# nadimkanazi/cacto

Measured on AMD Instinct MI355X. Metric: env-steps/sec + critic-updates/sec per node, double_integrator & manipulator, higher is better.
Workload: dtype f32 (MLP, MFMA) / f64 (dynamics)

## Files before the change

### cacto_amd/csrc/rollout_kernels.hip

```cpp
#include <cstdlib>
#include <utility>

#include "net_common.h"

#ifdef CACTO_STAMPS
__device__ unsigned long long g_rstamps[20];
__device__ unsigned long long g_ttacc[1024 * 2 * 2 * 10];
__device__ unsigned long long g_wsacc[1024 * 8 * 7];
#define RSTAMP(k)                                                                     \
  do {                                                                                \
    if (blockIdx.x == 0 && threadIdx.x == 0 && it == 20) g_rstamps[k] = __builtin_amdgcn_s_memtime(); \
  } while (0)
#else
#define RSTAMP(k) \
  do {            \
  } while (0)
#endif

namespace cacto {

template <typename F, int... I>
__device__ __forceinline__ void static_for_impl(F&& f, std::integer_sequence<int, I...>) {
  (f(std::integral_constant<int, I>{}), ...);
}
// ... 884 lines not shown
        const double* s = sr.s;
#pragma unroll
        for (int i = 0; i < na; ++i) {
          a[i] = use_actor ? Sh.W.a[c * na + i] : 0.f;
          ad[i] = (double)a[i];
        }
        if constexpr (NJ > 0) {
          if (split_dyn) {
            double M[NJ * NJ], h[NJ];
#pragma unroll
            for (int k = 0; k < NJ * NJ; ++k) M[k] = Sh.MS[k * SL + c];
#pragma unroll
            for (int i = 0; i < NJ; ++i) h[i] = Sh.hS[i * SL + c];
            chain_step<NJ>(sd, s, ad, M, h, sn);
          } else if (NJ == 3 && planar) {
            planar3_step(Planar3(sd.pl), ks.dt, s, ad, sn);
          } else {
            ro_simulate<NJ>(ks, sr.cd, s, ad, sn);
          }
        } else {
          ro_simulate<NJ>(ks, sr.cd, s, ad, sn);
        }
        RSTAMP(6);
#pragma unroll
        for (int i = 0; i < ns; ++i) {
          Sh.sS[c * ns + i] = sn[i];
          sr.s[i] = sn[i];
        }
      }
      constexpr bool EARLY = NJ >= 3;
      if constexpr (EARLY) {
        __builtin_amdgcn_fence(__ATOMIC_ACQ_REL, "wavefront");
        x0l.write(Sh, nrm, L.lane);
      }
      RSTAMP(16);
      if (active) {
        fin = ro_advance<NJ, NG>(c, sr.b, sr.t, sr.s, a, sd, T, Straj, Atraj, status, nrm, sr.n);
        sr.t += 1;
        RSTAMP(7);
      }
      ro_refill<NJ, NG>(fin, c, head, Sh, sd, S0, nsteps, order, T, B, G, Straj, status, nrm, L, (int)blockIdx.x);
      if (fin) sr.load(Sh, c, cdyn);
      if constexpr (!EARLY) {
        __builtin_amdgcn_fence(__ATOMIC_ACQ_REL, "wavefront");
        x0l.write(Sh, nrm, L.lane);
      }
      const uint64_t m = __ballot(L.lane < SL && Sh.sact[c]);
      if (L.lane == 0) Sh.anyact = m != 0;
      RSTAMP(8);
    }
    __syncthreads();
    RSTAMP(3);
  }
}

struct RoSplitTT {
  static constexpr int REGK = 128, LDSK = 128;
};

template <int NA>
struct RoTeamActorLds {
  static constexpr int SL = 4;
  float h1[4 * RoCfg<1>::H1B];
  float h2[SL * RoCfg<1>::H2S];
  float x0[64];
  float a[SL * NA];
};

template <int NJ>
struct RoTeamShared {
  static constexpr int ns = Dims<NJ>::NS, na = Dims<NJ>::NA, SL = 4;
  RoTeamActorLds<na> W;
  double sS[SL * ns];
  double MS[NJ > 0 ? SL * NJ * NJ : 1], hS[NJ > 0 ? SL * NJ : 1];
  int sb[SL], sn[SL], st[SL], sact[SL];
  int anyact;
  int bar;
};

template <int NJ>
struct RoTTShared {
  static constexpr int na = Dims<NJ>::NA;
  float4 w2[RoSplitTT::LDSK / 4 * 4 * 64];
  float w3[na * 256];
  float b3[8];
  RoTeamShared<NJ> team[2];
};

template <int NA>
struct RoTeamView {
  const float4* w2;
  const float* w3;
  const float* b3;
  float* h1;
  float* h2;
  float* x0;
  float* a;
};

#ifndef RO_TBAR_SLEEP
#define RO_TBAR_SLEEP 1
#endif
struct RoTeamBar {
  int* ctr;
  int target;
  int lane;
  __device__ __forceinline__ void operator()() {
    target += 4;
    if (lane == 0) __hip_atomic_fetch_add(ctr, 1, __ATOMIC_RELEASE, __HIP_MEMORY_SCOPE_WORKGROUP);
    while (__hip_atomic_load(ctr, __ATOMIC_ACQUIRE, __HIP_MEMORY_SCOPE_WORKGROUP) < target)
      __builtin_amdgcn_s_sleep(RO_TBAR_SLEEP);
  }
};

template <int NJ>
__global__ void __launch_bounds__(2 * CACTO_THREADS, 1)
    k_rollout_tt(const SysDevice* __restrict__ sdp, NetView N, const double* __restrict__ S0,
                 const int32_t* __restrict__ nsteps, int T, int use_actor, double* __restrict__ Straj,
                 float* __restrict__ Atraj, int32_t* __restrict__ status, const int32_t* __restrict__ order, int B) {
  constexpr int ns = Dims<NJ>::NS, na = Dims<NJ>::NA, NG = 1, SL = 4;
  constexpr int REGK = RoSplitTT::REGK, LDSK = RoSplitTT::LDSK;
  __shared__ RoTTShared<NJ> Sh;
  const SysDevice& sd = *sdp;
  const cacto_sys_params& p = sd.p;
  const int team = threadIdx.x >> 8;
  Lane L;
  L.wave = (L.wave + team) & 3;
  L.tid = L.wave * 64 + L.lane;
  RoTeamShared<NJ>& S = Sh.team[team];
  RoActorRegs<ns, REGK> R;
  if (use_actor) {
    const float* W1 = N.flat + N.t.woff[0];
    const float* W2 = N.flat + N.t.woff[1];
    const float* W3 = N.flat + N.t.woff[2];
    const int f = 64 * L.wave + L.lane;
#pragma unroll
    for (int k = 0; k < REGK; ++k) R.w2[k] = W2[k * 256 + f];
#pragma unroll
    for (int q = 0; q < ns; ++q) R.w1[q] = W1[q * 256 + f];
    R.b1 = N.bias(0, f);
    R.b2 = N.bias(1, f);
    for (int e = threadIdx.x; e < LDSK * 64; e += 2 * CACTO_THREADS) {
      const int lane = e & 63, w = (e >> 6) & 3, kq = e >> 8;
      const int k = REGK + 4 * kq, col = 64 * w + lane;
      Sh.w2[e] = make_float4(W2[k * 256 + col], W2[(k + 1) * 256 + col], W2[(k + 2) * 256 + col],
                             W2[(k + 3) * 256 + col]);
    }
    for (int e = threadIdx.x; e < na * 256; e += 2 * CACTO_THREADS) Sh.w3[e] = W3[(e & 255) * na + (e >> 8)];
    if (threadIdx.x < 8) Sh.b3[threadIdx.x] = threadIdx.x < na ? N.bias(2, threadIdx.x) : 0.f;
  }
  if (L.tid < 64) S.W.x0[L.tid] = 0.f;
  for (int e = L.tid; e < SL * ns; e += CACTO_THREADS) S.sS[e] = 0.0;
  if (L.tid < SL) S.sact[L.tid] = 0;
  if (L.tid == 0) S.bar = 0;
  __syncthreads();
  RoTeamBar tbar{&S.bar, 0, L.lane};
  const int vb = 2 * (int)blockIdx.x + team, G = 2 * (int)gridDim.x;
  int head = 0;
  const RoNorm<ns> nrm(p);
  const RoSimScalars ks{p.dt, p.L_delta, p.tau_delta};
  const int c = L.lane % SL;
  ConstDyn<NJ> cd;
  if constexpr (NJ > 0) {
#pragma unroll
    for (int k = 0; k < NJ * NJ; ++k) cd.L[k] = sd.cd_L[k];
#pragma unroll
    for (int i = 0; i < NJ; ++i) cd.h[i] = sd.cd_h[i];
  }
  RoSlotRegs<NJ, NG> sr;
  if (L.wave == 0) {
    ro_refill<NJ, NG, RoTeamShared<NJ>, false>(L.lane < SL, L.lane, head, S, sd, S0, nsteps, order, T, B, G, Straj,
                                                status, nrm, L, vb);
    const uint64_t m = __ballot(L.lane < SL && S.sact[L.lane]);
    if (L.lane == 0) S.anyact = m != 0;
    sr.load(S, c, false);
  }
  tbar();
  const RoX0Lane<ns, SL> x0l(nrm, L.lane);
  RoTeamView<na> V{Sh.w2, Sh.w3, Sh.b3, S.W.h1, S.W.h2, S.W.x0, S.W.a};
  const float* W2g = N.flat + N.t.woff[1];
#ifdef CACTO_STAMPS
#define TSTAMP(k)                                                                                          \
  do {                                                                                                     \
    if (blockIdx.x == 0 && L.wave == 0 && L.lane == 0 && it == 20) g_rstamps[8 * team + k] = __builtin_amdgcn_s_memtime(); \
  } while (0)
  unsigned long long tacc[9] = {0, 0, 0, 0, 0, 0, 0, 0, 0}, tprev = 0, tsub = 0;
  int tbi = 0;
  auto tmark = [&](int ph) {
    const unsigned long long now = __builtin_amdgcn_s_memtime();
    if (ph == 1) tacc[0] += now - tprev;
    if (ph == 2) tacc[1] += now - tprev;
    if (ph == 3) tacc[2] += now - tprev;
    if (ph == 4) tacc[3] += now - tprev;
    if (ph == 5) tacc[4] += now - tprev;
    tprev = now;
    tsub = now;
  };
  auto tsubmark = [&](int k) {
    const unsigned long long now = __builtin_amdgcn_s_memtime();
    if (k == 5) tacc[5] += now - tsub;
    if (k == 6) tacc[6] += now - tsub;
    if (k == 7) tacc[7] += now - tsub;
    if (k == 8) tacc[8] += now - tsub;
    tsub = now;
  };
#define TSUB(k) tsubmark(k)
  auto sbar = [&] {
    tbar();
    tmark(++tbi);
  };
  int tsteps = 0;
#else
#define TSTAMP(k) \
  do {            \
  } while (0)
#define TSUB(k) \
  do {          \
  } while (0)
#endif
  for (int it = 0; S.anyact; ++it) {
    TSTAMP(0);
    if (!use_actor) tbar();
#ifdef CACTO_STAMPS
    tbi = 0;
    tmark(0);
    if (use_actor) ro_actor<NG, ns, na, REGK, LDSK, true, true>(R, V, W2g, L, it, sbar);
#else
    if (use_actor) ro_actor<NG, ns, na, REGK, LDSK, true, true>(R, V, W2g, L, it, tbar);
#endif
    TSTAMP(1);
    if (L.wave == 0) {
      const bool active = L.lane < SL && sr.act;
      bool fin = false;
      float a[na];
      if (active) {
        double ad[na], sn[ns];
#pragma unroll
        for (int i = 0; i < na; ++i) {
          a[i] = use_actor ? S.W.a[c * na + i] : 0.f;
          ad[i] = (double)a[i];
        }
        ro_simulate<NJ>(ks, cd, sr.s, ad, sn);
#pragma unroll
        for (int i = 0; i < ns; ++i) {
          S.sS[c * ns + i] = sn[i];
          sr.s[i] = sn[i];
        }
      }
      TSUB(5);
      if (active) {
        fin = ro_advance<NJ, NG>(c, sr.b, sr.t, sr.s, a, sd, T, Straj, Atraj, status, nrm, sr.n);
        sr.t += 1;
      }
      TSUB(6);
      ro_refill<NJ, NG, RoTeamShared<NJ>, false>(fin, c, head, S, sd, S0, nsteps, order, T, B, G, Straj, status, nrm,
                                                  L, vb);
      if (fin) sr.load(S, c, false);
      TSUB(7);
      __builtin_amdgcn_fence(__ATOMIC_ACQ_REL, "wavefront");
      x0l.write(S, nrm, L.lane);
      const uint64_t m = __ballot(L.lane < SL && S.sact[c]);
      if (L.lane == 0) S.anyact = m != 0;
      TSUB(8);
      TSTAMP(2);
    }
#ifdef CACTO_STAMPS
    tmark(4);
#endif
    tbar();
    TSTAMP(3);
#ifdef CACTO_STAMPS
    tmark(5);
    ++tsteps;
#endif
  }
#ifdef CACTO_STAMPS
  if (L.lane == 0 && L.wave < 2) {
    unsigned long long* o = g_ttacc + ((size_t)(blockIdx.x * 2 + team) * 2 + L.wave) * 10;
    for (int k = 0; k < 9; ++k) o[k] = tacc[k];
    o[9] = tsteps;
  }
#endif
#undef TSTAMP
#undef TSUB
}

template <int N, typename V>
__device__ __forceinline__ V lane_pick(const V* x, int lane) {
  V v = x[0];
#pragma unroll
  for (int i = 1; i < N; ++i) {
    v = lane == i ? x[i] : v;
    __asm__ volatile("" : "+v"(v));
  }
  return v;
}

__device__ __forceinline__ double readlane_d(double v, int l) {
  const long long b = __double_as_longlong(v);
  const int lo = __builtin_amdgcn_readlane((int)b, l), hi = __builtin_amdgcn_readlane((int)(b >> 32), l);
  return __longlong_as_double(((long long)hi << 32) | (unsigned)lo);
}

template <int NJ>
struct RoKsShared {
  float h1[2 * 4 * RoCfg<1>::H1B];
  float P[2][8 * 256];
  int act[8];
  int qhead;
  static constexpr bool LW = NJ == 3;
  float w3s[LW ? 3 * 256 : 1];
  float b2s[LW ? 256 : 1];
  float4 w1s[LW ? 8 * 64 : 1];
  double pls[LW ? 20 : 1];
};

template <int NJ>
__global__ void __launch_bounds__(8 * CACTO_WAVE, 1)
    k_rollout_ks(const SysDevice* __restrict__ sdp, NetView N, const double* __restrict__ S0,
                 const int32_t* __restrict__ nsteps, int T, int use_actor, double* __restrict__ Straj,
                 float* __restrict__ Atraj, int32_t* __restrict__ status, const int32_t* __restrict__ order, int B) {
  constexpr int ns = Dims<NJ>::NS, na = Dims<NJ>::NA;
  constexpr int H1B = RoCfg<1>::H1B;
  __shared__ RoKsShared<NJ> Sh;
  const SysDevice& sd = *sdp;
  const cacto_sys_params& p = sd.p;
  const int w = threadIdx.x >> 6, lane = threadIdx.x & 63;
  const int fq = w & 3, hk = w >> 2;
  const int sg = w >> 2, si = w & 3;
  constexpr bool LW = RoKsShared<NJ>::LW;
  float w2[128], b2[LW ? 1 : 4], w1[LW ? 1 : ns][4], b1[LW ? 1 : 4], w3[LW ? 1 : na][4], b3[na];
  if (use_actor) {
    const float* W1 = N.flat + N.t.woff[0];
    const float* W2 = N.flat + N.t.woff[1];
    const float* W3 = N.flat + N.t.woff[2];
#pragma unroll
    for (int k = 0; k < 128; ++k) w2[k] = W2[(128 * hk + k) * 256 + 64 * fq + lane];
#pragma unroll
    for (int m = 0; m < 4; ++m) {
      if constexpr (!LW) {
#pragma unroll
        for (int q = 0; q < ns; ++q) w1[q][m] = W1[q * 256 + lane + 64 * m];
        b1[m] = N.bias(0, lane + 64 * m);
        b2[m] = N.bias(1, lane + 64 * m);
#pragma unroll
        for (int a = 0; a < na; ++a) w3[a][m] = W3[(lane + 64 * m) * na + a];
      }
    }
#pragma unroll
    for (int a = 0; a < na; ++a) b3[a] = N.bias(2, a);
    if constexpr (LW) {
      for (int e = threadIdx.x; e < na * 256; e += 8 * CACTO_WAVE) Sh.w3s[e] = W3[(e & 255) * na + (e >> 8)];
      for (int e = threadIdx.x; e < 256; e += 8 * CACTO_WAVE) Sh.b2s[e] = N.bias(1, e);
      for (int e = threadIdx.x; e < 8 * 64; e += 8 * CACTO_WAVE) {
        const int q = e >> 6, l = e & 63;
        float4 v;
        if (q < ns)
          v = make_float4(W1[q * 256 + l], W1[q * 256 + l + 64], W1[q * 256 + l + 128], W1[q * 256 + l + 192]);
        else
          v = make_float4(N.bias(0, l), N.bias(0, l + 64), N.bias(0, l + 128), N.bias(0, l + 192));
        Sh.w1s[e] = v;
      }
    }
  }
  if constexpr (LW)
    if (threadIdx.x < 20) Sh.pls[threadIdx.x] = sd.pl[threadIdx.x];
  for (int e = threadIdx.x; e < 2 * 4 * H1B; e += 8 * CACTO_WAVE) Sh.h1[e] = 0.f;
  if (threadIdx.x == 0) Sh.qhead = 0;
  __syncthreads();
  const int vb = (int)blockIdx.x, G = (int)gridDim.x;
  const RoNorm<ns> nrm(p);
  float nl = 1.f;
#pragma unroll
  for (int q = 0; q < ns; ++q) nl = lane == q ? nrm.n[q] : nl;
  const bool tl = lane == ns - 1;
  ConstDyn<NJ> cd;
  if constexpr (NJ > 0 && NJ != 3) {
#pragma unroll
    for (int k = 0; k < NJ * NJ; ++k) cd.L[k] = sd.cd_L[k];
#pragma unroll
    for (int i = 0; i < NJ; ++i) cd.h[i] = sd.cd_h[i];
  }
  const RoSimScalars ks{p.dt, p.L_delta, p.tau_delta};
  bool act = false;
  int b = 0, n = 0, t = 0;
  double s[ns];
#pragma unroll
  for (int i = 0; i < ns; ++i) s[i] = 0.0;

  auto refill = [&]() {
    act = false;
    while (true) {
      int k = 0;
      if (lane == 0) k = __hip_atomic_fetch_add(&Sh.qhead, 1, __ATOMIC_RELAXED, __HIP_MEMORY_SCOPE_WORKGROUP);
      k = __builtin_amdgcn_readfirstlane(k);
      const int r = k * G + ((k & 1) ? G - 1 - vb : vb);
      if (r >= B) return;
      const int bb = __builtin_amdgcn_readfirstlane(order ? order[r] : r);
      const int nn = min(nsteps[bb], T);
#pragma unroll
      for (int i = 0; i < ns; ++i) s[i] = S0[(size_t)bb * ns + i];
      if (Straj && lane < ns) Straj[(size_t)bb * (T + 1) * ns + lane] = lane_pick<ns>(s, lane);
      if (nn == 0) {
        if (status && lane == 0) status[bb] = 0;
        continue;
      }
      b = bb;
      n = nn;
      t = 0;
      act = true;
      return;
    }
  };
  auto layer1 = [&]() {
    const double sv = lane_pick<ns>(s, lane);
    const float qv = fdiv((float)sv, nl);
    const float xv = nrm.on ? (tl ? fsub(fmul(qv, 2.0f), 1.0f) : qv) : (float)sv;
    float x0[ns];
#pragma unroll
    for (int q = 0; q < ns; ++q) x0[q] = __int_as_float(__builtin_amdgcn_readlane(__float_as_int(xv), q));
    if constexpr (LW) {
      float4 wq[ns + 1];
#pragma unroll
      for (int q = 0; q <= ns; ++q) wq[q] = Sh.w1s[(q < ns ? q : 7) * 64 + lane];
#pragma unroll
      for (int m = 0; m < 4; ++m) {
        float acc = 0.f;
#pragma unroll
        for (int q = 0; q < ns; ++q) acc = __builtin_fmaf(x0[q], get4(wq[q], m), acc);
        Sh.h1[(sg * 4 + m) * H1B + (lane & 15) * 20 + 4 * si + (lane >> 4)] = lrelu(fadd(acc, get4(wq[ns], m)));
      }
    } else {
#pragma unroll
      for (int m = 0; m < 4; ++m) {
        float acc = 0.f;
#pragma unroll
        for (int q = 0; q < ns; ++q) acc = __builtin_fmaf(x0[q], w1[q][m], acc);
        Sh.h1[(sg * 4 + m) * H1B + (lane & 15) * 20 + 4 * si + (lane >> 4)] = lrelu(fadd(acc, b1[m]));
      }
    }
  };

#ifdef CACTO_STAMPS
  unsigned long long wacc[6] = {0, 0, 0, 0, 0, 0}, wprev = __builtin_amdgcn_s_memtime();
  int wsteps = 0;
  auto wmark = [&](int ph) {
    const unsigned long long now = __builtin_amdgcn_s_memtime();
#pragma unroll
    for (int k = 0; k < 6; ++k)
      if (k == ph) wacc[k] += now - wprev;
    wprev = now;
  };
#define KMARK(k) wmark(k)
#else
#define KMARK(k) \
  do {           \
  } while (0)
#endif

  refill();
  if (act && use_actor) layer1();
  if (lane == 0) Sh.act[w] = act;
  __syncthreads();
  const int rd = (lane >> 2) * 20 + 4 * (lane & 3);
  for (int it = 0;; ++it) {
    int any = 0;
#pragma unroll
    for (int k = 0; k < 8; ++k) any |= Sh.act[k];
    if (any == 0) break;
    if (!use_actor) __syncthreads();
    float a[na];
#pragma unroll
    for (int i = 0; i < na; ++i) a[i] = 0.f;
    if (use_actor) {
      float4 xa[2][2];
#pragma unroll
      for (int gg = 0; gg < 2; ++gg)
#pragma unroll
        for (int kl = 0; kl < 2; ++kl)
          xa[gg][kl] = *reinterpret_cast<const float4*>(&Sh.h1[(gg * 4 + 2 * hk + kl) * H1B + rd]);
      floatx4 acc[2][2];
#pragma unroll
      for (int gg = 0; gg < 2; ++gg) acc[gg][0] = acc[gg][1] = floatx4{0.f, 0.f, 0.f, 0.f};
#pragma unroll
      for (int kl = 0; kl < 2; ++kl)
#pragma unroll
        for (int v = 0; v < 4; ++v)
          static_for<16>([&](auto qc) {
            constexpr int q = decltype(qc)::value;
#pragma unroll
            for (int gg = 0; gg < 2; ++gg)
              acc[gg][q & 1] = mfma_bc<q>(get4(xa[gg][kl], v), w2[64 * kl + 16 * v + q], acc[gg][q & 1]);
          });
#pragma unroll
      for (int gg = 0; gg < 2; ++gg)
#pragma unroll
        for (int i = 0; i < 4; ++i) Sh.P[hk][(4 * gg + i) * 256 + 64 * fq + lane] = fadd(acc[gg][0][i], acc[gg][1][i]);
      __syncthreads();
      KMARK(0);
      if (act) {
        float pa[na];
#pragma unroll
        for (int i = 0; i < na; ++i) pa[i] = 0.f;
#pragma unroll
        for (int m = 0; m < 4; ++m) {
          const int f = lane + 64 * m;
          const float h = lrelu(fadd(fadd(Sh.P[0][w * 256 + f], Sh.P[1][w * 256 + f]), LW ? Sh.b2s[f] : b2[m % (LW ? 1 : 4)]));
#pragma unroll
          for (int i = 0; i < na; ++i) pa[i] = fmaf(LW ? Sh.w3s[i * 256 + f] : w3[LW ? 0 : i][m], h, pa[i]);
        }
        if constexpr (na == 2) {
          const auto r32 = __builtin_amdgcn_permlane32_swap(__float_as_uint(pa[0]), __float_as_uint(pa[1]), false, false);
          float v = __uint_as_float(r32[0]) + __uint_as_float(r32[1]);
          const auto r16 = __builtin_amdgcn_permlane16_swap(__float_as_uint(v), __float_as_uint(v), false, false);
          v = __uint_as_float(r16[0]) + __uint_as_float(r16[1]);
#pragma unroll
          for (int off = 8; off >= 1; off >>= 1) v = add_from_above(v, off);
          a[0] = fadd(__int_as_float(__builtin_amdgcn_readlane(__float_as_int(v), 0)), b3[0]);
          a[1] = fadd(__int_as_float(__builtin_amdgcn_readlane(__float_as_int(v), 32)), b3[1 % na]);
        } else if constexpr (na == 3) {
          const auto r32 = __builtin_amdgcn_permlane32_swap(__float_as_uint(pa[0]), __float_as_uint(pa[1]), false, false);
          const auto q32 = __builtin_amdgcn_permlane32_swap(__float_as_uint(pa[2]), __float_as_uint(pa[2]), false, false);
          float v = __uint_as_float(r32[0]) + __uint_as_float(r32[1]);
          float v2 = __uint_as_float(q32[0]) + __uint_as_float(q32[1]);
          const auto r16 = __builtin_amdgcn_permlane16_swap(__float_as_uint(v), __float_as_uint(v), false, false);
          const auto q16 = __builtin_amdgcn_permlane16_swap(__float_as_uint(v2), __float_as_uint(v2), false, false);
          v = __uint_as_float(r16[0]) + __uint_as_float(r16[1]);
          v2 = __uint_as_float(q16[0]) + __uint_as_float(q16[1]);
#pragma unroll
          for (int off = 8; off >= 1; off >>= 1) {
            v = add_from_above(v, off);
            v2 = add_from_above(v2, off);
          }
          a[0] = fadd(__int_as_float(__builtin_amdgcn_readlane(__float_as_int(v), 0)), b3[0]);
          a[1] = fadd(__int_as_float(__builtin_amdgcn_readlane(__float_as_int(v), 32)), b3[1 % na]);
          a[2 % na] = fadd(__int_as_float(__builtin_amdgcn_readlane(__float_as_int(v2), 0)), b3[2 % na]);
        } else {
#pragma unroll
          for (int off = 32; off >= 1; off >>= 1)
#pragma unroll
            for (int i = 0; i < na; ++i) pa[i] = add_from_above(pa[i], off);
#pragma unroll
          for (int i = 0; i < na; ++i)
            a[i] = __int_as_float(__builtin_amdgcn_readfirstlane(__float_as_int(fadd(pa[i], b3[i]))));
        }
      }
      KMARK(1);
    }
    bool fin = false;
    if (act) {
      double ad[na], sn[ns];
#pragma unroll
      for (int i = 0; i < na; ++i) ad[i] = (double)a[i];
      if constexpr (NJ == 3) {
        double sv, cv;
        joint_sincos((lane & 1) ? s[2] : s[1], &sv, &cv);
        planar3_step_sc(Planar3(Sh.pls), ks.dt, s, ad, readlane_d(sv, 0), readlane_d(cv, 0), readlane_d(sv, 1),
                        readlane_d(cv, 1), sn);
      } else
        ro_simulate<NJ>(ks, cd, s, ad, sn);
      bool bad = false;
#pragma unroll
      for (int i = 0; i < ns; ++i) bad |= isnan(sn[i]);
      if (Atraj && lane < na) Atraj[((size_t)b * T + t) * na + lane] = lane_pick<na>(a, lane);
      if (Straj && lane < ns) Straj[((size_t)b * (T + 1) + t + 1) * ns + lane] = lane_pick<ns>(sn, lane);
      if (bad && Straj) {
        for (int e = lane; e < (n - t - 1) * ns; e += 64)
          Straj[((size_t)b * (T + 1) + t + 2) * ns + e] = __builtin_nan("");
      }
      fin = bad || t + 1 >= n;
      if (fin && status && lane == 0) status[b] = bad ? 1 : 0;
#pragma unroll
      for (int i = 0; i < ns; ++i) s[i] = sn[i];
      t += 1;
    }
    KMARK(2);
    if (fin) refill();
    KMARK(3);
    if (act && use_actor) layer1();
    if (lane == 0) Sh.act[w] = act;
    KMARK(4);
    __syncthreads();
    KMARK(5);
#ifdef CACTO_STAMPS
    ++wsteps;
#endif
  }
#ifdef CACTO_STAMPS
  if (lane == 0) {
    unsigned long long* o = g_wsacc + ((size_t)blockIdx.x * 8 + w) * 7;
    for (int k = 0; k < 6; ++k) o[k] = wacc[k];
    o[6] = wsteps;
  }
#endif
#undef KMARK
}

template <int NJ>
__global__ void __launch_bounds__(256, 4) k_rollout_rewards(const SysDevice* __restrict__ sdp, const double* __restrict__ Straj,
                                                         const float* __restrict__ Atraj, const int32_t* __restrict__ nsteps,
                                                         int T, int use_actor, const double* __restrict__ Wext,
                                                         double* __restrict__ Rtraj, double* __restrict__ EEtraj, int B) {
  constexpr int ns = Dims<NJ>::NS, na = Dims<NJ>::NA;
  const SysDevice& sd = *sdp;
  const int64_t total = (int64_t)B * (T + 1);
  double w[8];
#pragma unroll
  for (int k = 0; k < 8; ++k) w[k] = k >= sd.p.n_weights ? 0.0 : Wext ? Wext[k] : sd.p.w_running[k];
  for (int64_t e = blockIdx.x * (int64_t)blockDim.x + threadIdx.x; e < total; e += (int64_t)gridDim.x * blockDim.x) {
    const int b = (int)(e / (T + 1)), t = (int)(e % (T + 1));
    const int n = min(nsteps[b], T);
    if (t > n) continue;
    double s[ns];
    bool bad = false;
#pragma unroll
    for (int i = 0; i < ns; ++i) {
      s[i] = Straj[(size_t)e * ns + i];
      bad |= isnan(s[i]);
    }
    if (bad) continue;
    const V3 v = env_ee<NJ>(sd, s);
    if (EEtraj) {
      EEtraj[(size_t)e * 3 + 0] = v.x;
      EEtraj[(size_t)e * 3 + 1] = v.y;
      EEtraj[(size_t)e * 3 + 2] = v.z;
    }
    if (Rtraj && t < n) {
      double a[na];
#pragma unroll
      for (int i = 0; i < na; ++i) a[i] = use_actor ? (double)Atraj[((size_t)b * T + t) * na + i] : 0.0;
      Rtraj[(size_t)b * T + t] = env_reward_at<NJ>(sd, w, s, a, false, v);
    }
  }
}

#define CACTO_REW_SCAN_MAX 16000
template <int NJ>
__global__ void __launch_bounds__(256, 4) k_rollout_rewards_c(const SysDevice* __restrict__ sdp,
                                                           const double* __restrict__ Straj,
                                                           const float* __restrict__ Atraj,
                                                           const int32_t* __restrict__ nsteps, int T, int use_actor,
                                                           const double* __restrict__ Wext, double* __restrict__ Rtraj,
                                                           double* __restrict__ EEtraj, int B) {
  constexpr int ns = Dims<NJ>::NS, na = Dims<NJ>::NA;
  extern __shared__ int offs[];
  __shared__ int wsum[4];
  const SysDevice& sd = *sdp;
  const int tid = threadIdx.x, lane = tid & 63, wv = tid >> 6;
  const int per = (B + 255) / 256, b0 = tid * per;
  int loc = 0;
  for (int k = 0; k < per; ++k) {
    const int b = b0 + k;
    if (b < B) {
      const int n = min(nsteps[b], T);
      loc += n >= 0 ? n + 1 : 0;
    }
  }
  int inc = loc;
#pragma unroll
  for (int d = 1; d < 64; d <<= 1) {
    const int o = __shfl_up(inc, d);
    if (lane >= d) inc += o;
  }
  if (lane == 63) wsum[wv] = inc;
  __syncthreads();
  int base = 0;
  for (int w = 0; w < wv; ++w) base += wsum[w];
  int run = base + inc - loc;
  for (int k = 0; k < per; ++k) {
    const int b = b0 + k;
    if (b < B) {
      offs[b] = run;
      const int n = min(nsteps[b], T);
      run += n >= 0 ? n + 1 : 0;
    }
  }
  if (tid == 255) offs[B] = base + inc;
  __syncthreads();
  const int total = offs[B];
  double w[8];
#pragma unroll
  for (int k = 0; k < 8; ++k) w[k] = k >= sd.p.n_weights ? 0.0 : Wext ? Wext[k] : sd.p.w_running[k];
  for (int e = blockIdx.x * 256 + tid; e < total; e += gridDim.x * 256) {
    int lo = 0, hi = B;
    while (hi - lo > 1) {
      const int mid = (lo + hi) >> 1;
      if (offs[mid] <= e) lo = mid;
      else hi = mid;
    }
    const int b = lo, t = e - offs[b];
    const int n = min(nsteps[b], T);
    const size_t row = (size_t)b * (T + 1) + t;
    double s[ns];
    bool bad = false;
#pragma unroll
    for (int i = 0; i < ns; ++i) {
      s[i] = Straj[row * ns + i];
      bad |= isnan(s[i]);
    }
    if (bad) continue;
    const V3 v = env_ee<NJ>(sd, s);
    if (EEtraj) {
      EEtraj[row * 3 + 0] = v.x;
      EEtraj[row * 3 + 1] = v.y;
      EEtraj[row * 3 + 2] = v.z;
    }
    if (Rtraj && t < n) {
      double a[na];
#pragma unroll
      for (int i = 0; i < na; ++i) a[i] = use_actor ? (double)Atraj[((size_t)b * T + t) * na + i] : 0.0;
      Rtraj[(size_t)b * T + t] = env_reward_at<NJ>(sd, w, s, a, false, v);
    }
  }
}

inline int ro_cus() {
  static int cus = 0;
  if (cus == 0) {
    int dev = 0, v = 0;
    if (hipGetDevice(&dev) == hipSuccess && hipDeviceGetAttribute(&v, hipDeviceAttributeMultiprocessorCount, dev) == hipSuccess && v > 0)
      cus = v;
    else
      cus = 256;
  }
  return cus;
}

}

using namespace cacto;

namespace {
template <int NJ>
struct LaunchRolloutRewards {
  static int run(const cacto_sys* sys, const double* S, const float* A, const int32_t* n, int T, int use_actor,
                 const double* W, double* R, double* EE, int B, hipStream_t st) {
    const int64_t total = (int64_t)B * (T + 1);
    static const char* force = std::getenv("CACTO_REW_GRID");
    const bool compact = force ? force[0] == 'c' : NJ == -2;
    if (B <= CACTO_REW_SCAN_MAX && compact) {
      const int grid = (int)std::max<int64_t>(1, std::min<int64_t>((total + 255) / 256, 4 * ro_cus()));
      hipLaunchKernelGGL(k_rollout_rewards_c<NJ>, dim3(grid), dim3(256), (size_t)(B + 1) * sizeof(int), st, sys->dev,
                         S, A, n, T, use_actor, W, R, EE, B);
    } else {
      const int grid = (int)std::max<int64_t>(1, std::min<int64_t>((total + 255) / 256, 8 * ro_cus()));
      hipLaunchKernelGGL(k_rollout_rewards<NJ>, dim3(grid), dim3(256), 0, st, sys->dev, S, A, n, T, use_actor, W, R,
                         EE, B);
    }
    CACTO_CHECK_HIP(hipGetLastError());
    return CACTO_OK;
  }
};

template <int NJ>
struct LaunchRollout {
  static int run(const cacto_sys* sys, NetView v, const double* S0, const int32_t* n, int T, int use_actor,
                 const double* W, double* S, float* A, double* R, double* EE, int32_t* status, const int32_t* order,
                 int B, int groups, int wgs, hipStream_t st) {
    const int cus = ro_cus();
    constexpr bool tt_ok = NJ <= 2 && !(NJ > 0 && !RoConstDyn<NJ>::ok);
    const bool tt_sys = tt_ok && (NJ <= 0 || sys->host.p.const_dyn);
    const bool tt_auto = tt_sys && NJ > 0;
    constexpr bool ks_ok = tt_ok || NJ == 3;
    const bool planar = NJ == 3 && sys->host.pl[0] != 0.0;
    const bool ks_sys = tt_sys || planar;
    if ((groups == -1 && !tt_sys) || (groups == -3 && !ks_sys)) {
      set_error("cacto_rollout_sched: groups -1 needs a system without configuration-dependent M, -3 such a system "
                "or a planar 3-joint chain");
      return CACTO_EINVAL;
    }
    const bool ks_auto = (tt_sys && B <= 2 * 8 * cus) || planar;
    if (groups == -3 || (groups == 0 && ks_auto)) {
      if (wgs <= 0) wgs = std::min(cus, ceil_div(B, 8));
      wgs = std::max(1, std::min(wgs, ceil_div(B, 8)));
      if constexpr (ks_ok)
        hipLaunchKernelGGL(k_rollout_ks<NJ>, dim3(wgs), dim3(8 * CACTO_WAVE), 0, st, sys->dev, v, S0, n, T,
                           use_actor, S, A, status, order, B);
      CACTO_CHECK_HIP(hipGetLastError());
      if (R || EE) return LaunchRolloutRewards<NJ>::run(sys, S, A, n, T, use_actor, W, R, EE, B, st);
      return CACTO_OK;
    }
    if (tt_sys && (groups == -1 || (tt_auto && groups == 0 && B / (2 * 4 * cus) == 2))) {
      if (wgs <= 0) wgs = std::min(cus, ceil_div(B, 8));
      wgs = std::max(1, std::min(wgs, ceil_div(B, 8)));
      if constexpr (tt_ok)
        hipLaunchKernelGGL(k_rollout_tt<NJ>, dim3(wgs), dim3(2 * CACTO_THREADS), 0, st, sys->dev, v, S0, n, T,
                           use_actor, S, A, status, order, B);
      CACTO_CHECK_HIP(hipGetLastError());
      if (R || EE) return LaunchRolloutRewards<NJ>::run(sys, S, A, n, T, use_actor, W, R, EE, B, st);
      return CACTO_OK;
    }
    constexpr int gmax = 4;
    if (groups <= 0) {
      const int per = B / (2 * 4 * cus);
      groups = std::min(gmax, per >= 4 ? 4 : per >= 2 ? 2 : 1);
    }
    if (groups > gmax) {
      set_error("cacto_rollout_sched: groups above this system's maximum (1 for 6 joints)");
      return CACTO_EINVAL;
    }
    if (wgs <= 0) wgs = std::min(cus, ceil_div(B, 4 * groups));
    wgs = std::max(1, std::min(wgs, ceil_div(B, 4 * groups)));
    switch (groups) {
      case 1:
        hipLaunchKernelGGL((k_rollout<NJ, 1>), dim3(wgs), dim3(CACTO_THREADS), 0, st, sys->dev, v, S0, n, T, use_actor,
                           S, A, status, order, B);
        break;
      case 2:
        hipLaunchKernelGGL((k_rollout<NJ, (gmax >= 2 ? 2 : 1)>), dim3(wgs), dim3(CACTO_THREADS), 0, st, sys->dev, v, S0,
                           n, T, use_actor, S, A, status, order, B);
        break;
      case 4:
        hipLaunchKernelGGL((k_rollout<NJ, (gmax >= 4 ? 4 : 1)>), dim3(wgs), dim3(CACTO_THREADS), 0, st, sys->dev, v, S0,
                           n, T, use_actor, S, A, status, order, B);
        break;
      default:
        set_error("cacto_rollout_sched: groups must be 1, 2 or 4");
        return CACTO_EINVAL;
    }
    CACTO_CHECK_HIP(hipGetLastError());
    if (R || EE) return LaunchRolloutRewards<NJ>::run(sys, S, A, n, T, use_actor, W, R, EE, B, st);
    return CACTO_OK;
  }
};
}

#ifdef CACTO_STAMPS
extern "C" int cacto_debug_rollout_stamps(unsigned long long* out_h) {
  CACTO_CHECK_HIP(hipDeviceSynchronize());
  CACTO_CHECK_HIP(hipMemcpyFromSymbol(out_h, HIP_SYMBOL(g_rstamps), sizeof(unsigned long long) * 20));
  return CACTO_OK;
}
extern "C" int cacto_debug_rollout_ws_acc(unsigned long long* out_h) {
  CACTO_CHECK_HIP(hipDeviceSynchronize());
  CACTO_CHECK_HIP(hipMemcpyFromSymbol(out_h, HIP_SYMBOL(g_wsacc), sizeof(unsigned long long) * 1024 * 8 * 7));
  return CACTO_OK;
}
extern "C" int cacto_debug_rollout_tt_acc(unsigned long long* out_h) {
  CACTO_CHECK_HIP(hipDeviceSynchronize());
  CACTO_CHECK_HIP(hipMemcpyFromSymbol(out_h, HIP_SYMBOL(g_ttacc), sizeof(unsigned long long) * 1024 * 2 * 2 * 10));
  return CACTO_OK;
}
#endif

extern "C" int cacto_rollout_sched(const cacto_sys* sys, const float* actor_netbuf_d, const double* S0_d,
                                   const int32_t* nsteps_d, int T, int use_actor, const double* W_d, double* S_traj_d,
                                   float* A_traj_d, double* R_traj_d, double* EE_traj_d, int32_t* status_d,
                                   const int32_t* order_d, int B, int groups, int workgroups, void* stream) {
  CACTO_REQUIRE(sys && S0_d && nsteps_d && T >= 0 && B >= 0, "cacto_rollout: bad arguments");
  CACTO_REQUIRE(!use_actor || actor_netbuf_d, "cacto_rollout: use_actor needs the actor net buffer");
  CACTO_REQUIRE(groups == 0 || groups == 1 || groups == 2 || groups == 4 || groups == -1 || groups == -3,
                "cacto_rollout_sched: groups must be 0, 1, 2, 4, -1 (two teams) or -3 (one slot per wave, layer 2 "
                "split over K)");
  CACTO_REQUIRE(workgroups >= 0, "cacto_rollout_sched: workgroups must be >= 0");
  CACTO_REQUIRE(!(R_traj_d || EE_traj_d) || (S_traj_d && (A_traj_d || !use_actor)),
                "cacto_rollout: R_traj / EE_traj need S_traj (and A_traj when use_actor)");
  if (B == 0) return CACTO_OK;
  NetView v = cacto_make_view(sys, CACTO_NET_ACTOR, actor_netbuf_d);
  return dispatch_nj<LaunchRollout>(sys->host.p, sys, v, S0_d, nsteps_d, T, use_actor, W_d, S_traj_d, A_traj_d,
                                    R_traj_d, EE_traj_d, status_d, order_d, B, groups, workgroups, as_stream(stream));
}

extern "C" int cacto_rollout_rewards(const cacto_sys* sys, const double* S_traj_d, const float* A_traj_d,
                                     const int32_t* nsteps_d, int T, int use_actor, const double* W_d,
                                     double* R_traj_d, double* EE_traj_d, int B, void* stream) {
  CACTO_REQUIRE(sys && S_traj_d && nsteps_d && T >= 0 && B >= 0, "cacto_rollout_rewards: bad arguments");
  CACTO_REQUIRE(!use_actor || A_traj_d, "cacto_rollout_rewards: use_actor needs A_traj");
  if (B == 0 || !(R_traj_d || EE_traj_d)) return CACTO_OK;
  return dispatch_nj<LaunchRolloutRewards>(sys->host.p, sys, S_traj_d, A_traj_d, nsteps_d, T, use_actor, W_d,
                                           R_traj_d, EE_traj_d, B, as_stream(stream));
}

extern "C" int cacto_rollout(const cacto_sys* sys, const float* actor_netbuf_d, const double* S0_d,
                             const int32_t* nsteps_d, int T, int use_actor, const double* W_d, double* S_traj_d,
                             float* A_traj_d, double* R_traj_d, double* EE_traj_d, int32_t* status_d,
                             const int32_t* order_d, int B, void* stream) {
  return cacto_rollout_sched(sys, actor_netbuf_d, S0_d, nsteps_d, T, use_actor, W_d, S_traj_d, A_traj_d, R_traj_d,
                             EE_traj_d, status_d, order_d, B, 0, 0, stream);
}
```

Baseline: 691.2 million.

## Add two-slots-per-wave variant of the K-split rollout kernel

Templates the K-split rollout kernel on slots per wave so each 64-lane wave holds two environments in its 32-lane halves. Layer-2 MFMA work loops over twice as many groups and the layer-3 reduction combines the two halves. Cross-lane reads are redirected per half. The variant is auto-selected for large batches on eligible systems. It doubles environments per workgroup so there are fewer workgroups and better amortization of the MFMA and weight loads, at the cost of more shared memory and serial per-step work per wave.

```diff
diff --git a/cacto_amd/csrc/rollout_kernels.hip b/cacto_amd/csrc/rollout_kernels.hip
--- a/cacto_amd/csrc/rollout_kernels.hip
+++ b/cacto_amd/csrc/rollout_kernels.hip
@@ -1210,33 +1210,53 @@
   return __longlong_as_double(((long long)hi << 32) | (unsigned)lo);
 }
 
-template <int NJ>
+template <int NJ, int SPW = 1>
 struct RoKsShared {
-  float h1[2 * 4 * RoCfg<1>::H1B];
-  float P[2][8 * 256];
-  int act[8];
+  float h1[SPW * 2 * 4 * RoCfg<1>::H1B];
+  float P[2][SPW * 8 * 256];
+  int act[SPW * 8];
   int qhead;
-  static constexpr bool LW = NJ == 3;
+  static constexpr bool LW = NJ == 3 || SPW == 2;
   float w3s[LW ? 3 * 256 : 1];
   float b2s[LW ? 256 : 1];
   float4 w1s[LW ? 8 * 64 : 1];
-  double pls[LW ? 20 : 1];
-};
-
-template <int NJ>
+  double pls[NJ == 3 ? 20 : 1];
+};
+
+template <int NJ, int SPW>
 __global__ void __launch_bounds__(8 * CACTO_WAVE, 1)
     k_rollout_ks(const SysDevice* __restrict__ sdp, NetView N, const double* __restrict__ S0,
                  const int32_t* __restrict__ nsteps, int T, int use_actor, double* __restrict__ Straj,
                  float* __restrict__ Atraj, int32_t* __restrict__ status, const int32_t* __restrict__ order, int B) {
+  static_assert(SPW == 1 || SPW == 2, "slots per wave");
   constexpr int ns = Dims<NJ>::NS, na = Dims<NJ>::NA;
   constexpr int H1B = RoCfg<1>::H1B;
-  __shared__ RoKsShared<NJ> Sh;
+  __shared__ RoKsShared<NJ, SPW> Sh;
   const SysDevice& sd = *sdp;
   const cacto_sys_params& p = sd.p;
   const int w = threadIdx.x >> 6, lane = threadIdx.x & 63;
   const int fq = w & 3, hk = w >> 2;
-  const int sg = w >> 2, si = w & 3;
-  constexpr bool LW = RoKsShared<NJ>::LW;
+  constexpr int HL = 64 / SPW;
+  const int hf = SPW == 2 ? lane >> 5 : 0, hl = SPW == 2 ? lane & 31 : lane;
+  const int sw = w + 8 * hf;
+  const int sg = sw >> 2, si = w & 3;
+  auto hb = [&](int v, int l) -> int {
+    if constexpr (SPW == 2) {
+      const int lo = __builtin_amdgcn_readlane(v, l), hi = __builtin_amdgcn_readlane(v, 32 + l);
+      return hf ? hi : lo;
+    } else
+      return __builtin_amdgcn_readlane(v, l);
+  };
+  auto hbf = [&](float v, int l) -> float { return __int_as_float(hb(__float_as_int(v), l)); };
+  auto hbd = [&](double v, int l) -> double {
+    if constexpr (SPW == 2) {
+      const double lo = readlane_d(v, l), hi = readlane_d(v, 32 + l);
+      return hf ? hi : lo;
+    } else
+      return readlane_d(v, l);
+  };
+  constexpr bool LW = RoKsShared<NJ, SPW>::LW;
+  static_assert(!LW || (ns <= 7 && na <= 3), "w1s / w3s rows");
   float w2[128], b2[LW ? 1 : 4], w1[LW ? 1 : ns][4], b1[LW ? 1 : 4], w3[LW ? 1 : na][4], b3[na];
   if (use_actor) {
     const float* W1 = N.flat + N.t.woff[0];
@@ -1271,17 +1291,17 @@
       }
     }
   }
-  if constexpr (LW)
+  if constexpr (NJ == 3)
     if (threadIdx.x < 20) Sh.pls[threadIdx.x] = sd.pl[threadIdx.x];
-  for (int e = threadIdx.x; e < 2 * 4 * H1B; e += 8 * CACTO_WAVE) Sh.h1[e] = 0.f;
+  for (int e = threadIdx.x; e < SPW * 2 * 4 * H1B; e += 8 * CACTO_WAVE) Sh.h1[e] = 0.f;
   if (threadIdx.x == 0) Sh.qhead = 0;
   __syncthreads();
   const int vb = (int)blockIdx.x, G = (int)gridDim.x;
   const RoNorm<ns> nrm(p);
   float nl = 1.f;
 #pragma unroll
-  for (int q = 0; q < ns; ++q) nl = lane == q ? nrm.n[q] : nl;
-  const bool tl = lane == ns - 1;
+  for (int q = 0; q < ns; ++q) nl = hl == q ? nrm.n[q] : nl;
+  const bool tl = hl == ns - 1;
   ConstDyn<NJ> cd;
   if constexpr (NJ > 0 && NJ != 3) {
 #pragma unroll
@@ -1300,17 +1320,18 @@
     act = false;
     while (true) {
       int k = 0;
-      if (lane == 0) k = __hip_atomic_fetch_add(&Sh.qhead, 1, __ATOMIC_RELAXED, __HIP_MEMORY_SCOPE_WORKGROUP);
-      k = __builtin_amdgcn_readfirstlane(k);
+      if (hl == 0) k = __hip_atomic_fetch_add(&Sh.qhead, 1, __ATOMIC_RELAXED, __HIP_MEMORY_SCOPE_WORKGROUP);
+      k = SPW == 2 ? hb(k, 0) : __builtin_amdgcn_readfirstlane(k);
       const int r = k * G + ((k & 1) ? G - 1 - vb : vb);
       if (r >= B) return;
-      const int bb = __builtin_amdgcn_readfirstlane(order ? order[r] : r);
+      const int br = order ? order[r] : r;
+      const int bb = SPW == 2 ? br : __builtin_amdgcn_readfirstlane(br);
       const int nn = min(nsteps[bb], T);
 #pragma unroll
       for (int i = 0; i < ns; ++i) s[i] = S0[(size_t)bb * ns + i];
-      if (Straj && lane < ns) Straj[(size_t)bb * (T + 1) * ns + lane] = lane_pick<ns>(s, lane);
+      if (Straj && hl < ns) Straj[(size_t)bb * (T + 1) * ns + hl] = lane_pick<ns>(s, hl);
       if (nn == 0) {
-        if (status && lane == 0) status[bb] = 0;
+        if (status && hl == 0) status[bb] = 0;
         continue;
       }
       b = bb;
@@ -1321,22 +1342,26 @@
     }
   };
   auto layer1 = [&]() {
-    const double sv = lane_pick<ns>(s, lane);
+    const double sv = lane_pick<ns>(s, hl);
     const float qv = fdiv((float)sv, nl);
     const float xv = nrm.on ? (tl ? fsub(fmul(qv, 2.0f), 1.0f) : qv) : (float)sv;
     float x0[ns];
 #pragma unroll
-    for (int q = 0; q < ns; ++q) x0[q] = __int_as_float(__builtin_amdgcn_readlane(__float_as_int(xv), q));
+    for (int q = 0; q < ns; ++q) x0[q] = hbf(xv, q);
     if constexpr (LW) {
-      float4 wq[ns + 1];
-#pragma unroll
-      for (int q = 0; q <= ns; ++q) wq[q] = Sh.w1s[(q < ns ? q : 7) * 64 + lane];
-#pragma unroll
-      for (int m = 0; m < 4; ++m) {
-        float acc = 0.f;
-#pragma unroll
-        for (int q = 0; q < ns; ++q) acc = __builtin_fmaf(x0[q], get4(wq[q], m), acc);
-        Sh.h1[(sg * 4 + m) * H1B + (lane & 15) * 20 + 4 * si + (lane >> 4)] = lrelu(fadd(acc, get4(wq[ns], m)));
+#pragma unroll
+      for (int c = 0; c < SPW; ++c) {
+        const int fl = hl + HL * c;
+        float4 wq[ns + 1];
+#pragma unroll
+        for (int q = 0; q <= ns; ++q) wq[q] = Sh.w1s[(q < ns ? q : 7) * 64 + fl];
+#pragma unroll
+        for (int m = 0; m < 4; ++m) {
+          float acc = 0.f;
+#pragma unroll
+          for (int q = 0; q < ns; ++q) acc = __builtin_fmaf(x0[q], get4(wq[q], m), acc);
+          Sh.h1[(sg * 4 + m) * H1B + (fl & 15) * 20 + 4 * si + (fl >> 4)] = lrelu(fadd(acc, get4(wq[ns], m)));
+        }
       }
     } else {
 #pragma unroll
@@ -1368,42 +1393,46 @@
 
   refill();
   if (act && use_actor) layer1();
-  if (lane == 0) Sh.act[w] = act;
+  if (hl == 0) Sh.act[sw] = act;
   __syncthreads();
   const int rd = (lane >> 2) * 20 + 4 * (lane & 3);
   for (int it = 0;; ++it) {
     int any = 0;
 #pragma unroll
-    for (int k = 0; k < 8; ++k) any |= Sh.act[k];
+    for (int k = 0; k < 8 * SPW; ++k) any |= Sh.act[k];
     if (any == 0) break;
     if (!use_actor) __syncthreads();
     float a[na];
 #pragma unroll
     for (int i = 0; i < na; ++i) a[i] = 0.f;
     if (use_actor) {
-      float4 xa[2][2];
-#pragma unroll
-      for (int gg = 0; gg < 2; ++gg)
+#pragma unroll 1
+      for (int g0 = 0; g0 < 2 * SPW; g0 += 2) {
+        float4 xa[2][2];
+#pragma unroll
+        for (int gg = 0; gg < 2; ++gg)
+#pragma unroll
+          for (int kl = 0; kl < 2; ++kl)
+            xa[gg][kl] = *reinterpret_cast<const float4*>(&Sh.h1[((g0 + gg) * 4 + 2 * hk + kl) * H1B + rd]);
+        floatx4 acc[2][2];
+#pragma unroll
+        for (int gg = 0; gg < 2; ++gg) acc[gg][0] = acc[gg][1] = floatx4{0.f, 0.f, 0.f, 0.f};
 #pragma unroll
         for (int kl = 0; kl < 2; ++kl)
-          xa[gg][kl] = *reinterpret_cast<const float4*>(&Sh.h1[(gg * 4 + 2 * hk + kl) * H1B + rd]);
-      floatx4 acc[2][2];
-#pragma unroll
-      for (int gg = 0; gg < 2; ++gg) acc[gg][0] = acc[gg][1] = floatx4{0.f, 0.f, 0.f, 0.f};
-#pragma unroll
-      for (int kl = 0; kl < 2; ++kl)
-#pragma unroll
-        for (int v = 0; v < 4; ++v)
-          static_for<16>([&](auto qc) {
-            constexpr int q = decltype(qc)::value;
-#pragma unroll
-            for (int gg = 0; gg < 2; ++gg)
-              acc[gg][q & 1] = mfma_bc<q>(get4(xa[gg][kl], v), w2[64 * kl + 16 * v + q], acc[gg][q & 1]);
-          });
-#pragma unroll
-      for (int gg = 0; gg < 2; ++gg)
-#pragma unroll
-        for (int i = 0; i < 4; ++i) Sh.P[hk][(4 * gg + i) * 256 + 64 * fq + lane] = fadd(acc[gg][0][i], acc[gg][1][i]);
+#pragma unroll
+          for (int v = 0; v < 4; ++v)
+            static_for<16>([&](auto qc) {
+              constexpr int q = decltype(qc)::value;
+#pragma unroll
+              for (int gg = 0; gg < 2; ++gg)
+                acc[gg][q & 1] = mfma_bc<q>(get4(xa[gg][kl], v), w2[64 * kl + 16 * v + q], acc[gg][q & 1]);
+            });
+#pragma unroll
+        for (int gg = 0; gg < 2; ++gg)
+#pragma unroll
+          for (int i = 0; i < 4; ++i)
+            Sh.P[hk][(4 * (g0 + gg) + i) * 256 + 64 * fq + lane] = fadd(acc[gg][0][i], acc[gg][1][i]);
+      }
       __syncthreads();
       KMARK(0);
       if (act) {
@@ -1412,12 +1441,32 @@
         for (int i = 0; i < na; ++i) pa[i] = 0.f;
 #pragma unroll
         for (int m = 0; m < 4; ++m) {
-          const int f = lane + 64 * m;
-          const float h = lrelu(fadd(fadd(Sh.P[0][w * 256 + f], Sh.P[1][w * 256 + f]), LW ? Sh.b2s[f] : b2[m % (LW ? 1 : 4)]));
+          const int f = hl + 64 * m;
+          const float h = lrelu(fadd(fadd(Sh.P[0][sw * 256 + f], Sh.P[1][sw * 256 + f]), LW ? Sh.b2s[f] : b2[m % (LW ? 1 : 4)]));
 #pragma unroll
           for (int i = 0; i < na; ++i) pa[i] = fmaf(LW ? Sh.w3s[i * 256 + f] : w3[LW ? 0 : i][m], h, pa[i]);
         }
-        if constexpr (na == 2) {
+        if constexpr (SPW == 2) {
+          float pb[na];
+#pragma unroll
+          for (int i = 0; i < na; ++i) pb[i] = 0.f;
+#pragma unroll
+          for (int m = 0; m < 4; ++m) {
+            const int f = hl + 32 + 64 * m;
+            const float h = lrelu(fadd(fadd(Sh.P[0][sw * 256 + f], Sh.P[1][sw * 256 + f]), Sh.b2s[f]));
+#pragma unroll
+            for (int i = 0; i < na; ++i) pb[i] = fmaf(Sh.w3s[i * 256 + f], h, pb[i]);
+          }
+#pragma unroll
+          for (int i = 0; i < na; ++i) {
+            float v = fadd(pa[i], pb[i]);
+            const auto r16 = __builtin_amdgcn_permlane16_swap(__float_as_uint(v), __float_as_uint(v), false, false);
+            v = __uint_as_float(r16[0]) + __uint_as_float(r16[1]);
+#pragma unroll
+            for (int off = 8; off >= 1; off >>= 1) v = add_from_above(v, off);
+            a[i] = fadd(hbf(v, 0), b3[i]);
+          }
+        } else if constexpr (na == 2) {
           const auto r32 = __builtin_amdgcn_permlane32_swap(__float_as_uint(pa[0]), __float_as_uint(pa[1]), false, false);
           float v = __uint_as_float(r32[0]) + __uint_as_float(r32[1]);
           const auto r16 = __builtin_amdgcn_permlane16_swap(__float_as_uint(v), __float_as_uint(v), false, false);
@@ -1463,21 +1512,22 @@
       if constexpr (NJ == 3) {
         double sv, cv;
         joint_sincos((lane & 1) ? s[2] : s[1], &sv, &cv);
-        planar3_step_sc(Planar3(Sh.pls), ks.dt, s, ad, readlane_d(sv, 0), readlane_d(cv, 0), readlane_d(sv, 1),
-                        readlane_d(cv, 1), sn);
+        planar3_step_sc(Planar3(Sh.pls), ks.dt, s, ad, hbd(sv, 0), hbd(cv, 0), hbd(sv, 1), hbd(cv, 1), sn);
       } else
         ro_simulate<NJ>(ks, cd, s, ad, sn);
       bool bad = false;
 #pragma unroll
       for (int i = 0; i < ns; ++i) bad |= isnan(sn[i]);
-      if (Atraj && lane < na) Atraj[((size_t)b * T + t) * na + lane] = lane_pick<na>(a, lane);
-      if (Straj && lane < ns) Straj[((size_t)b * (T + 1) + t + 1) * ns + lane] = lane_pick<ns>(sn, lane);
+      if (Atraj && hl < na) Atraj[((size_t)b * T + t) * na + hl] = lane_pick<na>(a, hl);
+      if (Straj && hl < ns) Straj[((size_t)b * (T + 1) + t + 1) * ns + hl] = lane_pick<ns>(sn, hl);
       if (bad && Straj) {
-        for (int e = lane; e < (n - t - 1) * ns; e += 64)
+        int e0 = hl;
+        if constexpr (SPW == 2) __asm__ volatile("" : "+v"(e0));
+        for (int e = e0; e < (n - t - 1) * ns; e += HL)
           Straj[((size_t)b * (T + 1) + t + 2) * ns + e] = __builtin_nan("");
       }
       fin = bad || t + 1 >= n;
-      if (fin && status && lane == 0) status[b] = bad ? 1 : 0;
+      if (fin && status && hl == 0) status[b] = bad ? 1 : 0;
 #pragma unroll
       for (int i = 0; i < ns; ++i) s[i] = sn[i];
       t += 1;
@@ -1486,7 +1536,7 @@
     if (fin) refill();
     KMARK(3);
     if (act && use_actor) layer1();
-    if (lane == 0) Sh.act[w] = act;
+    if (hl == 0) Sh.act[sw] = act;
     KMARK(4);
     __syncthreads();
     KMARK(5);
@@ -1661,6 +1711,11 @@
 };
 
 template <int NJ>
+struct RoKs2Auto {
+  static constexpr bool on = NJ == 3 || NJ == 2 || NJ == 0;
+};
+
+template <int NJ>
 struct LaunchRollout {
   static int run(const cacto_sys* sys, NetView v, const double* S0, const int32_t* n, int T, int use_actor,
                  const double* W, double* S, float* A, double* R, double* EE, int32_t* status, const int32_t* order,
@@ -1672,17 +1727,28 @@
     constexpr bool ks_ok = tt_ok || NJ == 3;
     const bool planar = NJ == 3 && sys->host.pl[0] != 0.0;
     const bool ks_sys = tt_sys || planar;
-    if ((groups == -1 && !tt_sys) || (groups == -3 && !ks_sys)) {
-      set_error("cacto_rollout_sched: groups -1 needs a system without configuration-dependent M, -3 such a system "
-                "or a planar 3-joint chain");
+    if ((groups == -1 && !tt_sys) || ((groups == -3 || groups == -4) && !ks_sys)) {
+      set_error("cacto_rollout_sched: groups -1 needs a system without configuration-dependent M, -3 / -4 such a "
+                "system or a planar 3-joint chain");
       return CACTO_EINVAL;
+    }
+    const bool ks2_auto = ks_sys && RoKs2Auto<NJ>::on && B >= 4 * 8 * cus;
+    if (groups == -4 || (groups == 0 && ks2_auto)) {
+      if (wgs <= 0) wgs = std::min(cus, ceil_div(B, 16));
+      wgs = std::max(1, std::min(wgs, ceil_div(B, 16)));
+      if constexpr (ks_ok)
+        hipLaunchKernelGGL((k_rollout_ks<NJ, 2>), dim3(wgs), dim3(8 * CACTO_WAVE), 0, st, sys->dev, v, S0, n, T,
+                           use_actor, S, A, status, order, B);
+      CACTO_CHECK_HIP(hipGetLastError());
+      if (R || EE) return LaunchRolloutRewards<NJ>::run(sys, S, A, n, T, use_actor, W, R, EE, B, st);
+      return CACTO_OK;
     }
     const bool ks_auto = (tt_sys && B <= 2 * 8 * cus) || planar;
     if (groups == -3 || (groups == 0 && ks_auto)) {
       if (wgs <= 0) wgs = std::min(cus, ceil_div(B, 8));
       wgs = std::max(1, std::min(wgs, ceil_div(B, 8)));
       if constexpr (ks_ok)
-        hipLaunchKernelGGL(k_rollout_ks<NJ>, dim3(wgs), dim3(8 * CACTO_WAVE), 0, st, sys->dev, v, S0, n, T,
+        hipLaunchKernelGGL((k_rollout_ks<NJ, 1>), dim3(wgs), dim3(8 * CACTO_WAVE), 0, st, sys->dev, v, S0, n, T,
                            use_actor, S, A, status, order, B);
       CACTO_CHECK_HIP(hipGetLastError());
       if (R || EE) return LaunchRolloutRewards<NJ>::run(sys, S, A, n, T, use_actor, W, R, EE, B, st);
@@ -1757,9 +1823,9 @@
                                    const int32_t* order_d, int B, int groups, int workgroups, void* stream) {
   CACTO_REQUIRE(sys && S0_d && nsteps_d && T >= 0 && B >= 0, "cacto_rollout: bad arguments");
   CACTO_REQUIRE(!use_actor || actor_netbuf_d, "cacto_rollout: use_actor needs the actor net buffer");
-  CACTO_REQUIRE(groups == 0 || groups == 1 || groups == 2 || groups == 4 || groups == -1 || groups == -3,
-                "cacto_rollout_sched: groups must be 0, 1, 2, 4, -1 (two teams) or -3 (one slot per wave, layer 2 "
-                "split over K)");
+  CACTO_REQUIRE(groups == 0 || groups == 1 || groups == 2 || groups == 4 || groups == -1 || groups == -3 || groups == -4,
+                "cacto_rollout_sched: groups must be 0, 1, 2, 4, -1 (two teams), -3 (one slot per wave, layer 2 "
+                "split over K) or -4 (the same with two slots per wave)");
   CACTO_REQUIRE(workgroups >= 0, "cacto_rollout_sched: workgroups must be >= 0");
   CACTO_REQUIRE(!(R_traj_d || EE_traj_d) || (S_traj_d && (A_traj_d || !use_actor)),
                 "cacto_rollout: R_traj / EE_traj need S_traj (and A_traj when use_actor)");
```

Result: no change. 691.7 million (median of 2 runs) (+0.1%).
